# PythonOptimizers/pysparse

Measured on AMD Instinct MI355X. Metric: CSR SpMV GB/s (7-pt Poisson, % of 8 TB/s HBM peak) + PCG iters/s, higher is better.
Workload: dtype f64

## Files before the change

### pysparse_amd/csrc/psp_csr_kernels.h

```cpp

constexpr int kBlock = 256;


__global__ void build_chunk_table(int nrows, const int *__restrict__ ind, int target, int nchunks,
                                  int2 *__restrict__ tab) {
  int c = blockIdx.x * blockDim.x + threadIdx.x;
  if (c > nchunks) return;
  int r;
  if (c == nchunks) {
    r = nrows;
  } else {
    long want = (long)c * target;
    int lo = 0, hi = nrows;
    while (lo < hi) {
      int mid = lo + ((hi - lo) >> 1);
      if ((long)ind[mid] >= want)
        hi = mid;
      else
        lo = mid + 1;
    }
    r = lo;
  }
  tab[c] = make_int2(r, ind[r]);
}
// ... 1040 lines not shown
      *reinterpret_cast<d2v *>(&buf[off + 2]) = p1[st];
    }
    __builtin_amdgcn_fence(__ATOMIC_SEQ_CST, "wavefront");
    __builtin_amdgcn_wave_barrier();
#pragma unroll
    for (int m = 0; m < NP; ++m) {
      const int i = 64 * m + lane;
      if (i < nr) {
        double acc = 0.0;
        for (int k = lo[m]; k < hi[m]; k += 8) {
          double t[8];
#pragma unroll
          for (int u = 0; u < 8; ++u) {
            int id = k + u;
            id = id < WT ? id : WT - 1;
            t[u] = buf[id];
          }
#pragma unroll
          for (int u = 0; u < 8; ++u) acc += (k + u < hi[m]) ? t[u] : 0.0;
        }
        if constexpr (NTS)
          __builtin_nontemporal_store(acc, &y[r0 + i]);
        else
          y[r0 + i] = acc;
        if (dotv) dsum += dotv[r0 + i] * acc;
      }
    }
  }
  if (partials) {
    dsum = wave_sum(dsum);
    __syncthreads();
    if (lane == 0) red[wid] = dsum;
    __syncthreads();
    if (threadIdx.x == 0) {
      double t = 0.0;
#pragma unroll
      for (int i = 0; i < WPB; ++i) t += red[i];
      partials[blockIdx.x] = t;
    }
  }
}

typedef double d2u __attribute__((ext_vector_type(2), aligned(8)));

constexpr int kDiaRows = 128;
constexpr int kDiaMaxOffs = 64;
constexpr int kDiaTable = 128;
constexpr int kDiaEmpty = -0x7fffffff - 1;

struct DiaOffs {
  int o[kDiaMaxOffs];
};

__global__ void dia_offsets_kernel(int nrows, const int *__restrict__ ind, const int *__restrict__ col,
                                   int *table, int *overflow) {
  for (int r = blockIdx.x * blockDim.x + threadIdx.x; r < nrows; r += gridDim.x * blockDim.x) {
    if (*(volatile int *)overflow) return;
    int prev = -1;
    for (int k = ind[r]; k < ind[r + 1]; ++k) {
      const int c = col[k];
      if (c <= prev) {
        *overflow = 1;
        return;
      }
      prev = c;
      const int o = c - r;
      unsigned h = ((unsigned)o * 2654435761u) >> 25;
      int probes = 0;
      for (; probes < kDiaTable; ++probes, h = (h + 1) & (kDiaTable - 1)) {
        int v = *(volatile int *)(table + h);
        if (v == o) break;
        if (v == kDiaEmpty) {
          v = atomicCAS(table + h, kDiaEmpty, o);
          if (v == kDiaEmpty || v == o) break;
        }
      }
      if (probes == kDiaTable) {
        *overflow = 1;
        return;
      }
    }
  }
}

template <typename MaskT>
__global__ void dia_build_kernel(int nrows, int no, DiaOffs offs, const int *__restrict__ ind,
                                 const int *__restrict__ col, const double *__restrict__ val,
                                 double *__restrict__ valT, MaskT *__restrict__ mask) {
  for (long r = (long)blockIdx.x * blockDim.x + threadIdx.x; r < nrows; r += (long)gridDim.x * blockDim.x) {
    const long blk = r / kDiaRows;
    const int i = (int)(r % kDiaRows);
    unsigned long long m = 0;
    for (int k = ind[r]; k < ind[r + 1]; ++k) {
      const int o = col[k] - (int)r;
      int b = 0;
      while (b < no - 1 && offs.o[b] != o) ++b;
      m |= 1ull << b;
      valT[((size_t)blk * no + b) * kDiaRows + i] = val[k];
    }
    mask[r] = (MaskT)m;
  }
}

__global__ void poisson_w4_kernel(int nx, int ny, int nz, long row_lo, long nloc, int no,
                                  double *__restrict__ valT, unsigned short *__restrict__ mask) {
  const long nxy = (long)nx * ny;
// ... 480 lines not shown
      for (int u = 0; u < G; ++u) {
        const int gu = g + u < no ? g + u : no - 1;
        og[u] = offs[gu];
        v[u] = ldg<true>(reinterpret_cast<const d2v *>(vp + (size_t)gu * kDiaRows));
        const long c = r + og[u];
        const long cc = c < 0 ? 0 : (c > cmax ? cmax : c);
        const d2u t = *reinterpret_cast<const d2u *>(x + cc);
        xv[u].x = t.x;
        xv[u].y = t.y;
        edge |= cc != c;
      }
      if (edge) {
#pragma unroll
        for (int u = 0; u < G; ++u) {
          const long c = r + og[u];
          if (c < 0 || c > cmax) {
            xv[u].x = (c >= 0 && c < ncols) ? x[c] : 0.0;
            xv[u].y = (c + 1 >= 0 && c + 1 < ncols) ? x[c + 1] : 0.0;
          }
        }
      }
#pragma unroll
      for (int u = 0; u < G; ++u) {
        const double t0 = a0 + v[u].x * xv[u].x;
        const double t1 = a1 + v[u].y * xv[u].y;
        const bool live = g + u < no;
        a0 = (live && ((m0 >> (g + u)) & 1ull)) ? t0 : a0;
        a1 = (live && ((m1 >> (g + u)) & 1ull)) ? t1 : a1;
      }
    }
    if (r + 1 < nrows) {
      d2u outu;
      outu.x = a0;
      outu.y = a1;
      __builtin_nontemporal_store(outu, reinterpret_cast<d2u *>(y + r));
      if (dotv) {
        const d2u u = *reinterpret_cast<const d2u *>(dotv + r);
        dsum += u.x * a0;
        dsum += u.y * a1;
      }
    } else {
      y[r] = a0;
      if (dotv) dsum += dotv[r] * a0;
    }
  }
  if (partials) {
    dsum = wave_sum(dsum);
    if (lane == 0) red[wid] = dsum;
    __syncthreads();
    if (threadIdx.x == 0) partials[blockIdx.x] = red[0] + red[1] + red[2] + red[3];
  }
}

template <int NO, int PRE, bool XU = false>
__global__ __launch_bounds__(256) void csr_spmv_w4_pf(
    int nrows, int stripe, DiaOffs offs, const double *__restrict__ valT,
    const unsigned short *__restrict__ mask, const double *__restrict__ r, const double *__restrict__ dinv,
    double dc, const double *__restrict__ p_old, double *__restrict__ p_new, double *__restrict__ q,
    double beta, int first, double *__restrict__ partials, const psp::PcgDev *__restrict__ dstate,
    double *__restrict__ x = nullptr, double *__restrict__ scan_partials = nullptr) {
  double alpha_x = 0.0;
  bool xp = false;
  if (dstate) {
    if (dstate->status) return;
    beta = dstate->beta;
    first = dstate->it == 1;
    if constexpr (XU) {
      alpha_x = dstate->alpha_x;
      xp = dstate->xpend != 0;
    }
  }
  __shared__ double red[4];
  __shared__ double red2[4];
  double dmax = 0.0;
  const int lane = threadIdx.x & 63;
  const int wid = __builtin_amdgcn_readfirstlane(threadIdx.x >> 6);
  int vb = (int)blockIdx.x;
  if (stripe > 0) {
    const int k = vb >> 3;
    vb = ((k / stripe) * 8 + (vb & 7)) * stripe + k % stripe;
  }
  const int blk = vb * 4 + wid;
  const long row = (long)blk * kDiaRows + 2 * lane;
  double dsum = 0.0;
  if (row < nrows) {
    const unsigned mm = *reinterpret_cast<const unsigned *>(mask + row);
    const unsigned m0 = mm & 0xffffu, m1 = mm >> 16;
    const double *vp = valT + (size_t)blk * NO * kDiaRows + 2 * lane;
    d2v v[NO];
#pragma unroll
    for (int o = 0; o < NO; ++o) v[o] = ldg<true>(reinterpret_cast<const d2v *>(vp + o * kDiaRows));
    const long cmax = (long)nrows - 2;
    const long rc = row > cmax ? cmax : row;
    d2u rr[NO + 1], pp[NO + 1], dd[NO + 1];
    bool edge = rc != row;
#pragma unroll
    for (int o = 0; o <= NO; ++o) {
      const long c = o < NO ? row + offs.o[o] : row;
      const long cc = c < 0 ? 0 : (c > cmax ? cmax : c);
      rr[o] = *reinterpret_cast<const d2u *>(r + cc);
      if (!first) pp[o] = *reinterpret_cast<const d2u *>(p_old + cc);
      if constexpr (PRE == 1) dd[o] = *reinterpret_cast<const d2u *>(dinv + cc);
      edge |= cc != c;
    }
    if (edge) {
#pragma unroll
      for (int o = 0; o <= NO; ++o) {
        const long c = o < NO ? row + offs.o[o] : row;
        if (c < 0 || c > cmax) {
          const bool i0 = c >= 0 && c < nrows, i1 = c + 1 >= 0 && c + 1 < nrows;
          rr[o].x = i0 ? r[c] : 0.0;
          rr[o].y = i1 ? r[c + 1] : 0.0;
          if (!first) {
            pp[o].x = i0 ? p_old[c] : 0.0;
            pp[o].y = i1 ? p_old[c + 1] : 0.0;
          }
          if constexpr (PRE == 1) {
            dd[o].x = i0 ? dinv[c] : 0.0;
            dd[o].y = i1 ? dinv[c + 1] : 0.0;
          }
        }
      }
    }
    d2v pn[NO + 1];
#pragma unroll
    for (int o = 0; o <= NO; ++o) {
      double z0 = rr[o].x, z1 = rr[o].y;
      if constexpr (PRE == 1) {
        z0 = z0 * dd[o].x;
        z1 = z1 * dd[o].y;
      }
      if constexpr (PRE == 2) {
        z0 = z0 * dc;
        z1 = z1 * dc;
      }
      if (!first) {
        z0 = z0 + beta * pp[o].x;
        z1 = z1 + beta * pp[o].y;
      }
      pn[o].x = z0;
      pn[o].y = z1;
    }
    double a0 = 0.0, a1 = 0.0;
#pragma unroll
// ... 237 lines not shown
```

### pysparse_amd/csrc/psp_csr_select.h

```cpp
namespace psp {

static int colmask() {
#ifdef PSP_TUNING
  static const int m = [] {
    const char *e = psp::tuning_env("PSP_SPMV_COLMASK");
    return e ? atoi(e) : -1;
  }();
  return m;
#else
  return -1;
#endif
}

static int spmv_stripe() {
  static const int m = [] {
    const char *e = psp::tuning_env("PSP_SPMV_STRIPE");
    return e ? atoi(e) : -1;
  }();
  return m;
}

static int w4_auto_stripe(const psp_csr *A) {
  if (A->sym_owner) return 32;
  int plane_wgs = 0;
// ... 188 lines not shown
  if (!on || !v.w4 || A->nparts || A->nrows != A->ncols || A->nrows < 2) return PSP_OK;
  const int stripe = w4_stripe(A, v);
  const int nblk = (A->nrows + kDiaRows - 1) / kDiaRows;
  const int grid = w4_grid(nblk, stripe);
  psp::CsrExtra *ex;
  {
    std::lock_guard<std::mutex> lk(g_extra_mu);
    ex = &g_extra[A];
  }
  bool sss = false;
  if (A->sym_owner) {
    psp_sss *S = const_cast<psp_sss *>(A->sym_owner);
    PSP_TRY(ensure_sss_w4(S));
    sss = S->w4_state == 1;
  }
  if (!sss) {
    PSP_TRY(ensure_w4(A, &ex));
    if (ex->dia_state != 1 || ex->dia_no > 16) return PSP_OK;
  }
  double *pbuf = partials;
  if (partials && grid > kMaxParts) {
    PSP_TRY(ensure_big_partials(ex, grid));
    pbuf = ex->big_partials;
  }
  if (sss)
    PSP_TRY(launch_sss_w4(A->sym_owner, stripe, x, y, x, pbuf, skip, grid, 1, xdiv, xdiv_dev));
  else
    PSP_TRY(launch_w4(A, ex, stripe, 0, nblk, x, y, x, pbuf, skip, grid, 1, xdiv, xdiv_dev));
  int np = grid;
  if (pbuf != partials) {
    np = kFold;
    hipLaunchKernelGGL(fold_partials_kernel, dim3(np / 16), dim3(256), 0, stream(), pbuf, grid, partials, np);
    PSP_LAUNCH_CHECK();
  }
  if (nparts) *nparts = np;
  *available = 1;
  return PSP_OK;
}

__global__ __launch_bounds__(256) void grid_wrap_check_kernel(int n, int nx, int ny, const unsigned short *__restrict__ mask,
                                                              int *__restrict__ bad) {
  int found = 0;
  for (long r = (long)blockIdx.x * blockDim.x + threadIdx.x; r < n; r += (long)gridDim.x * blockDim.x) {
    const unsigned m = mask[r];
    const int i = (int)(r % nx), j = (int)((r / nx) % ny);
    if (((m >> 2) & 1u) && i == 0) found = 1;
    if (((m >> 4) & 1u) && i == nx - 1) found = 1;
    if (((m >> 1) & 1u) && j == 0) found = 1;
    if (((m >> 5) & 1u) && j == ny - 1) found = 1;
  }
  if (found) atomicAdd(bad, 1);
}

__global__ __launch_bounds__(256) void w4_value_range_kernel(int n, int no, const double *__restrict__ valT,
                                                             const unsigned short *__restrict__ mask, double *__restrict__ out) {
  __shared__ double smin[4][16], smax[4][16];
  double lo[16], hi[16];
  for (int o = 0; o < 16; ++o) {
    lo[o] = INFINITY;
    hi[o] = -INFINITY;
  }
  for (long r = (long)blockIdx.x * blockDim.x + threadIdx.x; r < n; r += (long)gridDim.x * blockDim.x) {
    const unsigned m = mask[r];
    const double *vp = valT + (size_t)(r / kDiaRows) * no * kDiaRows + (size_t)(r % kDiaRows);
    for (int o = 0; o < no; ++o)
      if ((m >> o) & 1u) {
        const double v = vp[(size_t)o * kDiaRows];
        lo[o] = v < lo[o] ? v : lo[o];
        hi[o] = v > hi[o] ? v : hi[o];
        if (!(v == v)) hi[o] = INFINITY, lo[o] = -INFINITY;
      }
  }
  const int lane = threadIdx.x & 63, wid = threadIdx.x >> 6;
  for (int o = 0; o < no; ++o) {
    double a = lo[o], b = hi[o];
    for (int off = 32; off > 0; off >>= 1) {
      const double a2 = __shfl_down(a, off, 64), b2 = __shfl_down(b, off, 64);
      a = a2 < a ? a2 : a;
      b = b2 > b ? b2 : b;
    }
    if (lane == 0) {
      smin[wid][o] = a;
      smax[wid][o] = b;
    }
  }
  __syncthreads();
  if ((int)threadIdx.x < no) {
    const int o = threadIdx.x;
    double a = smin[0][o], b = smax[0][o];
    for (int w = 1; w < 4; ++w) {
      a = smin[w][o] < a ? smin[w][o] : a;
      b = smax[w][o] > b ? smax[w][o] : b;
    }
    out[((size_t)blockIdx.x * no + o) * 2] = a;
    out[((size_t)blockIdx.x * no + o) * 2 + 1] = b;
  }
}

int csr_w4_view(const psp_csr *A, W4View *out, int *available) {
  *available = 0;
  Variant v = decode_variant(A->variant);
  if (A->w4_only) v.w4 = true;
  if (!v.w4 || A->nparts || A->multi || A->host || A->nrows != A->ncols || A->nrows < 2) return PSP_OK;
  psp::CsrExtra *ex;
  PSP_TRY(ensure_w4(A, &ex));
  if (ex->dia_state != 1 || ex->dia_no > 9 || !ex->dia_mask) return PSP_OK;
  out->no = ex->dia_no;
  for (int i = 0; i < 12; ++i) out->offs[i] = i < ex->dia_no ? ex->dia_offs.o[i] : 0;
  out->valT = ex->dia_val;
  out->mask = ex->dia_mask;
  out->stripe = w4_stripe(A, v);
  out->grid = w4_grid((A->nrows + kDiaRows - 1) / kDiaRows, out->stripe);
  out->grid3[0] = out->grid3[1] = out->grid3[2] = 0;
  if (ex->dia_no == 7) {
    const int *o = out->offs;
    const int s1 = o[5], s2 = o[6];
    if (ex->grid_state < 0) {
      ex->grid_state = 0;
      if (o[3] == 0 && o[4] == 1 && o[2] == -1 && o[1] == -s1 && o[0] == -s2 && s1 >= 2 && s2 % s1 == 0 && s2 / s1 >= 2 &&
          A->nrows % s2 == 0 && A->nrows / s2 >= 2) {
        int *bad = nullptr;
        PSP_HIP(hipMalloc((void **)&bad, sizeof(int)));
        PSP_HIP(hipMemsetAsync(bad, 0, sizeof(int), stream()));
        hipLaunchKernelGGL(grid_wrap_check_kernel, dim3(std::min((A->nrows + 255) / 256, 4096)), dim3(256), 0, stream(),
                           A->nrows, s1, s2 / s1, ex->dia_mask, bad);
        int hbad = 1;
        const hipError_t e1 = hipMemcpyAsync(&hbad, bad, sizeof(int), hipMemcpyDeviceToHost, stream());
        const hipError_t e2 = hipStreamSynchronize(stream());
        (void)hipFree(bad);
        if (e1 != hipSuccess || e2 != hipSuccess) return fail(PSP_ENODEV, "csr_w4_view: grid check failed");
        if (hbad == 0) {
          ex->grid_state = 1;
          ex->grid_nx = s1;
          ex->grid_ny = s2 / s1;
        }
      }
    }
    if (ex->grid_state == 1) {
      out->grid3[0] = ex->grid_nx;
      out->grid3[1] = ex->grid_ny;
      out->grid3[2] = A->nrows / (ex->grid_nx * ex->grid_ny);
    }
  }
  out->constv = 0;
  if (ex->dia_no <= 12) {
    if (ex->constv_state < 0) {
      ex->constv_state = 0;
      const int no = ex->dia_no, blocks = std::min((A->nrows + 255) / 256, 512);
      double *d = nullptr;
      PSP_HIP(hipMalloc((void **)&d, sizeof(double) * 2 * no * blocks));
      hipLaunchKernelGGL(w4_value_range_kernel, dim3(blocks), dim3(256), 0, stream(), A->nrows, no, ex->dia_val, ex->dia_mask, d);
      std::vector<double> h((size_t)2 * no * blocks);
      const hipError_t e1 = hipMemcpyAsync(h.data(), d, sizeof(double) * h.size(), hipMemcpyDeviceToHost, stream());
      const hipError_t e2 = hipStreamSynchronize(stream());
      (void)hipFree(d);
      if (e1 != hipSuccess || e2 != hipSuccess) return fail(PSP_ENODEV, "csr_w4_view: value range pass failed");
      bool all = true;
      for (int o = 0; o < no && all; ++o) {
        double lo = INFINITY, hi = -INFINITY;
        for (int b = 0; b < blocks; ++b) {
          lo = std::min(lo, h[((size_t)b * no + o) * 2]);
          hi = std::max(hi, h[((size_t)b * no + o) * 2 + 1]);
        }
        if (!(lo == hi) || std::signbit(lo) != std::signbit(hi)) all = false;
        ex->constv[o] = lo;
      }
      if (all) ex->constv_state = 1;
    }
    if (ex->constv_state == 1) {
      out->constv = 1;
      for (int o = 0; o < 12; ++o) out->cval[o] = o < ex->dia_no ? ex->constv[o] : 0.0;
    }
  }
  *available = 1;
  return PSP_OK;
}

int csr_spmv_pfx_launch(const psp_csr *A, const double *r, const double *dinv, const double *p_old, double *p_new,
                        double *q, double *x, double *partials, int *nparts, const PcgDev *dstate, int *available) {
  *available = 0;
  Variant v = decode_variant(A->variant);
  if (!v.w4 || A->nparts || A->sym_owner || A->nrows != A->ncols || A->nrows < 2 || !dstate || !partials) return PSP_OK;
  psp::CsrExtra *ex;
  PSP_TRY(ensure_w4(A, &ex));
  if (ex->dia_state != 1 || ex->dia_no > 8) return PSP_OK;
  const int stripe = w4_stripe(A, v);
  const int nblk = (A->nrows + kDiaRows - 1) / kDiaRows;
  const int grid = w4_grid(nblk, stripe);
  if (grid > kMaxParts) return PSP_OK;
  double dc = 0.0;
  const int pre = !dinv ? 0 : (dinv_constant(dinv, A->nrows, &dc) ? 2 : 1);
  double *scan = partials + 2 * (size_t)kMaxParts;
#define PSP_PFX(NO, PRE)                                                                                    \
  hipLaunchKernelGGL((csr_spmv_w4_pf<NO, PRE, true>), dim3(grid), dim3(256), 0, stream(), A->nrows, stripe, \
                     ex->dia_offs, ex->dia_val, ex->dia_mask, r, dinv, dc, p_old, p_new, q, 0.0, 0, partials, dstate, x, scan)
#define PSP_PFX_NO(NO)                \
  case NO:                            \
    if (pre == 0) PSP_PFX(NO, 0);     \
    else if (pre == 1) PSP_PFX(NO, 1); \
    else PSP_PFX(NO, 2);              \
    break
  switch (ex->dia_no) {
    PSP_PFX_NO(1); PSP_PFX_NO(2); PSP_PFX_NO(3); PSP_PFX_NO(4); PSP_PFX_NO(5); PSP_PFX_NO(6); PSP_PFX_NO(7); PSP_PFX_NO(8);
    default:
      return PSP_OK;
  }
#undef PSP_PFX_NO
#undef PSP_PFX
  PSP_LAUNCH_CHECK();
  *nparts = grid;
  *available = 1;
  return PSP_OK;
}

bool csr_spmv_has_skip(const psp_csr *A) {
  if (A->nparts) {
    for (int p = 0; p < A->nparts; ++p)
      if (A->parts[p]->nrows && !csr_spmv_has_skip(A->parts[p])) return false;
    return true;
  }
  Variant v = decode_variant(A->variant);
  if (A->w4_only) v.w4 = true;
  if (v.w4 && A->sym_owner) {
    psp_sss *S = const_cast<psp_sss *>(A->sym_owner);
    if (ensure_sss_w4(S) != PSP_OK) return false;
    if (S->w4_state == 1) return true;
  }
  if (v.w4) {
    psp::CsrExtra *ex;
    if (ensure_w4(A, &ex) != PSP_OK) return false;
    if (ex->dia_state == 1) return true;
  }
  if (!v.w2 || A->max_row_nnz > v.tile / 2) return false;
  ChunkTable *t;
  if (get_chunk_table(const_cast<psp_csr *>(A), v.tile, &t) != PSP_OK) return false;
  if (ensure_rowoff(A, t) != PSP_OK) return false;
  return t->np != 0;
}

int csr_reordered_view(const psp_csr *A, psp_csr **R, const int **perm, const int **inv) {
  *R = nullptr;
  psp::setup_mark(nullptr);
  Variant v = decode_variant(A->variant);
  if (A->nparts || A->w4_only || A->no_reorder || !(v.w1 && v.w2 && v.w3) || A->nrows != A->ncols ||
      A->max_row_nnz > v.tile / 2 || v.tile != 1024)
    return PSP_OK;
  if (v.w4) {
    if (A->sym_owner) {
      psp_sss *S = const_cast<psp_sss *>(A->sym_owner);
      PSP_TRY(ensure_sss_w4(S));
      if (S->w4_state == 1) return PSP_OK;
    }
    psp::CsrExtra *ex;
    PSP_TRY(ensure_w4(A, &ex));
    if (ex->dia_state == 1) return PSP_OK;
  }
  psp::setup_mark("first use: index-free (w4) layouts tried");
  ChunkTable *t;
  PSP_TRY(get_chunk_table(const_cast<psp_csr *>(A), v.tile, &t));
  PSP_TRY(ensure_rowoff(A, t));
// ... 663 lines not shown
```

### pysparse_amd/csrc/psp_internal.h

```cpp
#pragma once
#include <hip/hip_runtime.h>

#include <algorithm>
#include <atomic>
#include <cstdarg>
#include <cstdint>
#include <cstdio>
#include <cstdlib>
#include <initializer_list>
#include <mutex>
#include <string>
#include <vector>

#include "pysparse_hip.h"
#include "psp_recur.h"

namespace psp {

int fail(int code, const char *fmt, ...) __attribute__((format(printf, 2, 3)));
const char *tuning_env(const char *name);
void note_solve(const char *loop, int launches_per_iter, int vec_bytes_per_row, int dinv_streamed);
void note_fallback();
bool single_kernel_loops_enabled();
void setup_mark(const char *label);
// ... 371 lines not shown
namespace psp {
struct PcgDev : PcgCol {
  int status;
  int xpend;
  int stag0;
  int head_rho0;
  int head_beta0;
  int pend_maxit;
  double alpha_x;
};
struct MinresDev : MinresRot {
  double norm_r0, errtol, relres;
  int status;
  int stop;
  int skip;
  int info, iter, it_max;
};
struct KryArg {
  const KryDev *S = nullptr;
  int i0 = 0, i1 = 0, i2 = 0;
};
int op_apply(const psp_op *op, const double *x_dev, double *y_dev);
int op_apply_block(const psp_op *op, int k, const double *X, long ldx, double *Y, long ldy, const int *frozen = nullptr);
int block_args(const char *what, int nrows, int ncols, int k, const double *X, long ldx, const double *Y, long ldy);
int csr_spmm_check(const char *what, const psp_csr *A);
int csr_spmm_launch(const psp_csr *A, int k, const double *X, long ldx, double *Y, long ldy, const int *skip,
                    double *partials, long pstride, int *nparts);
int jacobi_block_dev(const psp_jacobi *K, int k, const double *X, long ldx, double *Y, long ldy);
int robust_norm2(int n, const double *v, double sq, double *out);
int csr_spmv_launch_stored(const psp_csr *A, const double *x, double *y, const double *dotv, double *partials, int *nparts,
                           const int *skip = nullptr);
void batch_trim();
int correq_apply(const psp_op *op, const double *x_dev, double *y_dev);
int bv_tdot(long n, int m, const double *V, long ld, const double *x, double *h_dev);
int bv_gemv(long n, int m, const double *V, long ld, const double *h_dev, double alpha, double beta, double *y);
int bv_rotate(long n, int j, double *V, long ld, const double *U_host, int ldu, int u0, int jn, int dst0);
int bv_rotate_again(long n, int j, double *V, long ld, int jn, int dst0);
int bv_gram(long n, int ma, const double *A, long lda, int mb, const double *B, long ldb, double *G_dev, long ldg);
int bv_resid(long n, int k, const double *AX, long ldax, const double *MX, long ldmx, const double *theta_dev,
             const int *slot_host, double *R, long ldr, double *nrm2_dev);
void bv_trim();
void sym_jacobi_eig(int j, const double *Mu, int ldm, double *s, double *U, int ldu);
int random_fill_dev(long count, unsigned long long first, double *out);
int krylov_dev(int which, const psp_op *A, const psp_op *K, int n, double *x_dev, const double *b_dev, double tol, int maxit,
               int *info, int *iter, double *relres);
inline psp_csr *op_native_csr(const psp_op *op) {
  if (!op) return nullptr;
  if (op->kind == PSP_OP_CSR) return op->csr;
  if (op->kind == PSP_OP_SSS) return op->sss->full;
  return nullptr;
}
int csr_spmv_launch(const psp_csr *A, const double *x, double *y, const double *dotv,
                    double *partials, int *nparts, const int *skip = nullptr);
int csr_spmv_pfx_launch(const psp_csr *A, const double *r, const double *dinv, const double *p_old, double *p_new,
                        double *q, double *x, double *partials, int *nparts, const PcgDev *dstate, int *available);
int csr_spmv_scaled_launch(const psp_csr *A, const double *x, double xdiv, double *y, double *partials,
                           int *nparts, int *available, const int *skip = nullptr,
                           const double *xdiv_dev = nullptr);
int csr_reordered_view(const psp_csr *A, psp_csr **R, const int **perm, const int **inv);
int reorder_gather(int n, const int *perm_dev, const double *x, double *xp, const int *skip);
bool csr_spmv_has_skip(const psp_csr *A);
int csr_spmv_overlap(const psp_csr *A, const double *x, double *y, const double *dotv,
                     double *partials, int *nparts, int row_a, int row_b, int (*wait)(void *),
                     void *ctx, const int *skip = nullptr);
int dinv_register(const double *v, long n);
void dinv_unregister(const double *v);
bool dinv_constant(const double *v, long n, double *c);
int jacobi_apply_dev(psp_jacobi *K, const double *x, double *y);
struct W4View {
  int no;
  int offs[12];
  int grid3[3];
  int constv;
  double cval[12];
  const double *valT;
  const unsigned short *mask;
  int stripe, grid;
};
int csr_w4_view(const psp_csr *A, W4View *out, int *available);
constexpr int kCoopFallback = 1;
using PcgSkFn = int(const psp_csr *A, const double *dinv, int n, double *x, double *r, double *p, double *q, double n2b,
                     double tolb, double normr0, double rho0, int maxit, int *info, int *iter, double *relres, double *hist);
using MinresSkFn = int(const psp_csr *A, const double *dinv, int n, double *x, double *v_hat, double *y, double *w, double *v,
                        double *av, double norm_r0, double beta0, double errtol, int it_max, int *info, int *iter,
                        double *relres, double *hist);
bool mid_applicable(const psp_csr *A, int n);
bool mid_minres_applicable(const psp_csr *A, int n);
bool brick_applicable(const psp_csr *A, int n);
bool brick_minres_applicable(const psp_csr *A, int n);
bool coop_applicable(const psp_csr *A, int n);
PcgSkFn pcg_mid_loop, pcg_brick_loop, pcg_coop_loop;
MinresSkFn minres_mid_loop, minres_brick_loop, minres_coop_loop;
PcgSkFn *pcg_sk_choice(const psp_csr *A, int n, bool rho_nonzero);
int sk_capacity(const void *kernel, int block, size_t lds);

template <class Ctl>
struct SkLaunch {
  const void *kernel;
  int nwg, block;
  size_t lds;
  void **args;
  Ctl **ctl;
  double **part, **hist_dev;
  std::atomic<long long> *solves = nullptr, *fallbacks = nullptr;
};
struct SkVectors {
  int n;
  double *x, *stage;
// ... 117 lines not shown
```

### pysparse_amd/csrc/psp_solvers.hip

```cpp
#include <algorithm>
#include <array>
#include <cmath>
#include <cstdlib>
#include <cstring>
#include <initializer_list>
#include <type_traits>
#include <mutex>
#include <utility>
#include <vector>

#include "psp_internal.h"

using namespace psp;

namespace psp {
int k_dot(long n, const double *x, const double *y, double *partials, int *nparts);
int k_residual(long n, const double *b, double *r, const double *dinv, double *partials, int *nparts);
int k_pupdate(long n, const double *r, const double *dinv, double beta, bool first, double *p,
              const PcgDev *st = nullptr);
int k_px_update(long n, const double *r, const double *dinv, double *p, double *x, double *partials,
                int *nparts, const PcgDev *dstate, double beta = 0.0, double alpha = 0.0, bool first = false,
                bool xpend = false);
int k_x_update(long n, double alpha, const double *p, double *x, double *partials, int *nparts,
               const PcgDev *dstate);
// ... 415 lines not shown
  const double alpha = st->rho / pq;
  st->alpha = alpha;
  st->alpha_x = alpha;
  st->stag0 = alpha == 0.0 ? 1 : 0;
  st->xpend = 1;
}

__device__ __forceinline__ void pcg_lazy_scalar_r(PcgDev *st, const double *__restrict__ scal, double *__restrict__ hist) {
  if (st->status) return;
  const int it = st->it;
  const double normr = sqrt(scal[0]);
  st->normr = normr;
  if (hist) hist[it] = normr;
  if (normr <= st->tolb) {
    pcg_finish(st, 0, it);
  } else if (it == st->maxit) {
    st->pend_maxit = 1;
    st->status = 1;
  } else {
    const double rho1 = st->rho, rho = scal[1];
    st->rho1 = rho1;
    st->rho = rho;
    st->it = it + 1;
    st->head_rho0 = rho == 0.0 ? 1 : 0;
    st->head_beta0 = 0;
    if (rho != 0.0) {
      const double beta = rho / rho1;
      st->beta = beta;
      st->head_beta0 = beta == 0.0 ? 1 : 0;
    }
  }
}

struct PcgLazyXPq : StepOf<PcgDev, 1, true> {
  static __device__ void run(PcgDev *st, const double *v0, const double *v1, double *) {
    pcg_lazy_scalar_x(st, v0);
    pcg_lazy_scalar_pq(st, v1);
  }
};
struct PcgLazyR : StepOf<PcgDev> {
  static __device__ void run(PcgDev *st, const double *v, const double *, double *hist) { pcg_lazy_scalar_r(st, v, hist); }
};

static int pcg_lazy_enabled() {
  const char *e = psp::tuning_env("PSP_PCG_LAZYX");
  return e ? atoi(e) : 1;
}

static int pcg_lazypf_mode(int n) {
  const char *e = psp::tuning_env("PSP_PCG_LAZYPF");
  return e ? atoi(e) : (n >= (1 << 21) ? 1 : 0);
}

static int pcg_async_loop_lazy(psp_csr *Acsr, const double *dinv, int n, double *x, double *r, double *p, double *p2,
                               double *q, double n2b, double tolb, double normr0, double rho0, int maxit,
                               int *info, int *iter, double *relres, double *hist, bool *folded) {
  constexpr int kBatch = 16;
  double *const P[2] = {p, p2};
  int usepf = (p2 && pcg_lazypf_mode(n)) ? 1 : 0;
  *folded = false;
  Workspace *w;
  PSP_TRY(workspace(&w));
  LoopState<PcgDev> S;
  PSP_TRY(pcg_state_begin(S, n2b, tolb, normr0, rho0, maxit, hist != nullptr));
  PcgDev *st = S.dev;
  int enqueued = 0, np = 0;
  double *stag_parts = w->partials + 2 * (size_t)kMaxParts;
  do {
    const int batch = std::max(1, std::min(kBatch, maxit - enqueued));
    for (int i = 0; i < batch; ++i) {
      int np_x = 0;
      if (usepf) {
        const int e = enqueued + i + 1;
        PSP_TRY(csr_spmv_pfx_launch(Acsr, r, dinv, P[(e - 1) & 1], P[e & 1], q, x, w->partials, &np, st, &usepf));
        np_x = np;
      }
      if (!usepf) {
        PSP_TRY(k_px_update(n, r, dinv, p, x, w->partials, &np_x, st));
        PSP_TRY(csr_spmv_launch(Acsr, p, q, p, w->partials, &np, &st->status));
      }
      PSP_TRY(reduce2_then<PcgLazyXPq>(stag_parts, np_x, w->scal_dev + 8, w->partials, np, w->scal_dev, st, 2, 0));
      PSP_TRY(k_r_update(n, 0.0, q, dinv, r, w->partials, &np, st));
      PSP_TRY(reduce_then<PcgLazyR>(w->partials, np, 2, w->scal_dev + 4, st, S.hist));
    }
    enqueued += batch;
    PSP_TRY(S.fetch());
  } while (!S.host->status);
  *folded = usepf != 0;
  PcgDev *hst = S.host;
  if (usepf) p = P[hst->it & 1];
  if (hst->xpend) {
    double s[1];
    PSP_TRY(k_x_update(n, hst->alpha_x, p, x, w->partials, &np, nullptr));
    PSP_TRY(finish_partials(stag_parts, np, 1, w->scal_dev + 8));
    PSP_TRY(fetch_scalars(w->scal_dev + 8, 1, s));
    if (hst->pend_maxit) {
      const bool stag = hst->stag0 || s[0] == 0.0;
      hst->info = stag ? -5 : -1;
      hst->iter = stag ? maxit : maxit + 1;
      hst->relres = hst->normr / hst->n2b;
    }
  }
  *info = hst->info;
  *iter = hst->iter;
  *relres = hst->relres;
  if (hist) PSP_TRY(S.fetch_hist(hist, std::min(hst->iter, maxit)));
  return PSP_OK;
}

static bool norm2_unsafe(double sq) { return !(sq >= 1e-280 && sq <= 1e280); }
static int abs_max(int n, const double *v, double *out);
static int robust_nrm2(Workspace *w, int n, const double *v, double sq, double *out) {
  if (!norm2_unsafe(sq)) {
    *out = sqrt(sq);
    return PSP_OK;
  }
  double vmax = 0.0;
  PSP_TRY(abs_max(n, v, &vmax));
  if (vmax == 0.0 || vmax != vmax || std::isinf(vmax)) {
    *out = vmax == 0.0 ? 0.0 : sqrt(sq);
    return PSP_OK;
  }
  int e = 0;
  (void)frexp(vmax, &e);
  DevVecs mem;
  double *t;
  PSP_TRY(mem.alloc(n, &t));
  PSP_HIP(hipMemcpyAsync(t, v, sizeof(double) * (size_t)n, hipMemcpyDeviceToDevice, stream()));
  PSP_TRY(k_scal(n, ldexp(1.0, -e), t));
  int np;
  double s1;
  PSP_TRY(k_dot(n, t, t, w->partials, &np));
  PSP_TRY(reduce_fetch(w, np, 1, &s1));
  *out = ldexp(sqrt(s1), e);
  return PSP_OK;
}

namespace psp {
int robust_norm2(int n, const double *v, double sq, double *out) {
  Workspace *w;
  PSP_TRY(workspace(&w));
// ... 63 lines not shown
  PSP_TRY(robust_nrm2(w, n, b, s[0], &n2b));
  if (n2b == 0.0) {
    PSP_HIP(hipMemsetAsync(x, 0, sizeof(double) * (size_t)n, stream()));
    PSP_HIP(hipStreamSynchronize(stream()));
    *info = 0;
    *relres = 0.0;
    *iter = 0;
    return PSP_OK;
  }

  *info = -1;
  const double tolb = tol * n2b;

  if (Acsr_forced)
    PSP_TRY(csr_spmv_launch(Acsr, x, r, nullptr, nullptr, nullptr));
  else
    PSP_TRY(op_apply(A, x, r));
  PSP_TRY(k_residual(n, b, r, fused ? dinv : nullptr, w->partials, &np));
  PSP_TRY(reduce_fetch(w, np, 2, s));
  double normr;
  PSP_TRY(robust_nrm2(w, n, r, s[0], &normr));
  double rho_next = s[1];
  if (hist) hist[0] = normr;

  if (normr <= tolb) {
    *info = 0;
    *relres = normr / n2b;
    *iter = 0;
    return PSP_OK;
  }

  const bool sk = single_kernel_loops_enabled();
  double dcst;
  const int dstream = (dinv && !dinv_constant(dinv, n, &dcst)) ? 1 : 0;
  if (sk && fused && maxit >= 1)
    for (const PcgSkLoop &L : pcg_sk_loops()) {
      if ((L.needs_rho && rho_next == 0.0) || !L.applicable(Acsr, n)) continue;
      const int rc = L.run(Acsr, dinv, n, x, r, p, q, n2b, tolb, normr, rho_next, maxit, info, iter, relres, hist);
      if (rc != kCoopFallback) {
        note_solve(L.name, 1, 0, dstream);
        return rc;
      }
      note_fallback();
    }
  if (fused && maxit >= 1 && pcg_async_enabled() && csr_spmv_has_skip(Acsr)) {
    if (rho_next == 0.0) {
      *info = -2;
      *iter = 1;
      *relres = normr / n2b;
      return PSP_OK;
    }
    const int lazy_mode = pcg_lazy_enabled();
    const int rl = n > (1 << 21) ? 2 : 0;
    if (lazy_mode == 2 || (lazy_mode == 1 && (n < (1 << 24) || n >= 3 * (1 << 23)))) {
      bool pf = false;
      const int rc = pcg_async_loop_lazy(Acsr, dinv, n, x, r, p, p2, q, n2b, tolb, normr, rho_next, maxit, info, iter,
                                         relres, hist, &pf);
      note_solve(pf ? "pcg_lazy_pf" : "pcg_lazy", (pf ? 4 : 5) + rl, (pf ? 56 : 64) + 16 * dstream, dstream);
      return rc;
    }
    note_solve("pcg_eager", 6 + rl, 72 + 16 * dstream, dstream);
    return pcg_async_loop(Acsr, dinv, n, x, r, p, q, n2b, tolb, normr, rho_next, maxit, info, iter, relres, hist);
  }
  note_solve("pcg_host_scalars", -1, -1, dstream);

  PcgCol c = pcg_begin(n2b, tolb, normr, maxit);
  if (maxit < 1) pcg_exit(c, -1, 1);
  while (c.it <= maxit) {
    const double *zsrc = r;
    const double *zdinv = dinv;
    if (!fused) {
      zdinv = nullptr;
      if (K) {
        PSP_TRY(op_apply(K, r, z));
        zsrc = z;
      }
      PSP_TRY(k_dot(n, r, zsrc, w->partials, &np));
      PSP_TRY(reduce_fetch(w, np, 1, s));
      rho_next = s[0];
    }
    if (pcg_head(c, rho_next)) break;
    PSP_TRY(k_pupdate(n, zsrc, zdinv, c.it == 1 ? 0.0 : c.beta, c.it == 1, p));

    if (Acsr) {
      PSP_TRY(csr_spmv_launch(Acsr, p, q, p, w->partials, &np));
    } else {
      PSP_TRY(op_apply(A, p, q));
      PSP_TRY(k_dot(n, p, q, w->partials, &np));
    }
    PSP_TRY(reduce_fetch(w, np, 1, s));
    if (pcg_alpha(c, s[0])) break;

    PSP_TRY(k_xr_update(n, c.alpha, p, q, fused ? dinv : nullptr, x, r, w->partials, &np));
    PSP_TRY(reduce_fetch(w, np, 3, s));
    rho_next = s[1];
    const int it = c.it;
    const bool over = pcg_tail(c, sqrt(s[0]), s[2] == 0.0);
    if (hist) hist[it] = c.normr;
    if (over) break;
  }
  *info = c.info;
  *iter = c.iter;
  *relres = c.relres;
  PSP_HIP(hipStreamSynchronize(stream()));
  return PSP_OK;
}


struct PermutedSystem {
  psp_csr *R = nullptr;
  const int *perm = nullptr, *inv = nullptr;
// ... 1594 lines not shown
```

Before: 6113.

## Use constant stencil coefficients in fused PCG SpMV instead of streaming matrix values

```diff
diff --git a/pysparse_amd/csrc/psp_csr_kernels.h b/pysparse_amd/csrc/psp_csr_kernels.h
--- a/pysparse_amd/csrc/psp_csr_kernels.h
+++ b/pysparse_amd/csrc/psp_csr_kernels.h
@@ -1116,6 +1116,10 @@
   int o[kDiaMaxOffs];
 };
 
+struct DiaCVals {
+  double v[8];
+};
+
 __global__ void dia_offsets_kernel(int nrows, const int *__restrict__ ind, const int *__restrict__ col,
                                    int *table, int *overflow) {
   for (int r = blockIdx.x * blockDim.x + threadIdx.x; r < nrows; r += gridDim.x * blockDim.x) {
@@ -1702,9 +1706,9 @@
   }
 }
 
-template <int NO, int PRE, bool XU = false>
+template <int NO, int PRE, bool XU = false, bool CV = false>
 __global__ __launch_bounds__(256) void csr_spmv_w4_pf(
-    int nrows, int stripe, DiaOffs offs, const double *__restrict__ valT,
+    int nrows, int stripe, DiaOffs offs, DiaCVals cv, const double *__restrict__ valT,
     const unsigned short *__restrict__ mask, const double *__restrict__ r, const double *__restrict__ dinv,
     double dc, const double *__restrict__ p_old, double *__restrict__ p_new, double *__restrict__ q,
     double beta, int first, double *__restrict__ partials, const psp::PcgDev *__restrict__ dstate,
@@ -1736,10 +1740,15 @@
   if (row < nrows) {
     const unsigned mm = *reinterpret_cast<const unsigned *>(mask + row);
     const unsigned m0 = mm & 0xffffu, m1 = mm >> 16;
-    const double *vp = valT + (size_t)blk * NO * kDiaRows + 2 * lane;
     d2v v[NO];
-#pragma unroll
-    for (int o = 0; o < NO; ++o) v[o] = ldg<true>(reinterpret_cast<const d2v *>(vp + o * kDiaRows));
+    if constexpr (CV) {
+#pragma unroll
+      for (int o = 0; o < NO; ++o) v[o].x = v[o].y = cv.v[o];
+    } else {
+      const double *vp = valT + (size_t)blk * NO * kDiaRows + 2 * lane;
+#pragma unroll
+      for (int o = 0; o < NO; ++o) v[o] = ldg<true>(reinterpret_cast<const d2v *>(vp + o * kDiaRows));
+    }
     const long cmax = (long)nrows - 2;
     const long rc = row > cmax ? cmax : row;
     d2u rr[NO + 1], pp[NO + 1], dd[NO + 1];
diff --git a/pysparse_amd/csrc/psp_csr_select.h b/pysparse_amd/csrc/psp_csr_select.h
--- a/pysparse_amd/csrc/psp_csr_select.h
+++ b/pysparse_amd/csrc/psp_csr_select.h
@@ -264,6 +264,10 @@
   if (found) atomicAdd(bad, 1);
 }
 
+__host__ __device__ inline bool value_before(double a, double b) {
+  return a < b || (a == b && __builtin_signbit(a) && !__builtin_signbit(b));
+}
+
 __global__ __launch_bounds__(256) void w4_value_range_kernel(int n, int no, const double *__restrict__ valT,
                                                              const unsigned short *__restrict__ mask, double *__restrict__ out) {
   __shared__ double smin[4][16], smax[4][16];
@@ -278,8 +282,8 @@
     for (int o = 0; o < no; ++o)
       if ((m >> o) & 1u) {
         const double v = vp[(size_t)o * kDiaRows];
-        lo[o] = v < lo[o] ? v : lo[o];
-        hi[o] = v > hi[o] ? v : hi[o];
+        lo[o] = value_before(v, lo[o]) ? v : lo[o];
+        hi[o] = value_before(hi[o], v) ? v : hi[o];
         if (!(v == v)) hi[o] = INFINITY, lo[o] = -INFINITY;
       }
   }
@@ -288,8 +292,8 @@
     double a = lo[o], b = hi[o];
     for (int off = 32; off > 0; off >>= 1) {
       const double a2 = __shfl_down(a, off, 64), b2 = __shfl_down(b, off, 64);
-      a = a2 < a ? a2 : a;
-      b = b2 > b ? b2 : b;
+      a = value_before(a2, a) ? a2 : a;
+      b = value_before(b, b2) ? b2 : b;
     }
     if (lane == 0) {
       smin[wid][o] = a;
@@ -301,12 +305,43 @@
     const int o = threadIdx.x;
     double a = smin[0][o], b = smax[0][o];
     for (int w = 1; w < 4; ++w) {
-      a = smin[w][o] < a ? smin[w][o] : a;
-      b = smax[w][o] > b ? smax[w][o] : b;
+      a = value_before(smin[w][o], a) ? smin[w][o] : a;
+      b = value_before(b, smax[w][o]) ? smax[w][o] : b;
     }
     out[((size_t)blockIdx.x * no + o) * 2] = a;
     out[((size_t)blockIdx.x * no + o) * 2 + 1] = b;
   }
+}
+
+static int w4_const_values(const psp_csr *A, psp::CsrExtra *ex, bool *constv) {
+  *constv = false;
+  if (ex->dia_state != 1 || ex->dia_no > 12) return PSP_OK;
+  if (ex->constv_state < 0) {
+    ex->constv_state = 0;
+    const int no = ex->dia_no, blocks = std::min((A->nrows + 255) / 256, 512);
+    double *d = nullptr;
+    PSP_HIP(hipMalloc((void **)&d, sizeof(double) * 2 * no * blocks));
+    hipLaunchKernelGGL(w4_value_range_kernel, dim3(blocks), dim3(256), 0, stream(), A->nrows, no, ex->dia_val, ex->dia_mask, d);
+    std::vector<double> h((size_t)2 * no * blocks);
+    const hipError_t e1 = hipMemcpyAsync(h.data(), d, sizeof(double) * h.size(), hipMemcpyDeviceToHost, stream());
+    const hipError_t e2 = hipStreamSynchronize(stream());
+    (void)hipFree(d);
+    if (e1 != hipSuccess || e2 != hipSuccess) return fail(PSP_ENODEV, "w4_const_values: value range pass failed");
+    bool all = true;
+    for (int o = 0; o < no && all; ++o) {
+      double lo = INFINITY, hi = -INFINITY;
+      for (int b = 0; b < blocks; ++b) {
+        const double bl = h[((size_t)b * no + o) * 2], bh = h[((size_t)b * no + o) * 2 + 1];
+        lo = value_before(bl, lo) ? bl : lo;
+        hi = value_before(hi, bh) ? bh : hi;
+      }
+      if (!(lo == hi) || std::signbit(lo) != std::signbit(hi)) all = false;
+      ex->constv[o] = lo;
+    }
+    if (all) ex->constv_state = 1;
+  }
+  *constv = ex->constv_state == 1;
+  return PSP_OK;
 }
 
 int csr_w4_view(const psp_csr *A, W4View *out, int *available) {
@@ -354,70 +389,80 @@
       out->grid3[2] = A->nrows / (ex->grid_nx * ex->grid_ny);
     }
   }
-  out->constv = 0;
-  if (ex->dia_no <= 12) {
-    if (ex->constv_state < 0) {
-      ex->constv_state = 0;
-      const int no = ex->dia_no, blocks = std::min((A->nrows + 255) / 256, 512);
-      double *d = nullptr;
-      PSP_HIP(hipMalloc((void **)&d, sizeof(double) * 2 * no * blocks));
-      hipLaunchKernelGGL(w4_value_range_kernel, dim3(blocks), dim3(256), 0, stream(), A->nrows, no, ex->dia_val, ex->dia_mask, d);
-      std::vector<double> h((size_t)2 * no * blocks);
-      const hipError_t e1 = hipMemcpyAsync(h.data(), d, sizeof(double) * h.size(), hipMemcpyDeviceToHost, stream());
-      const hipError_t e2 = hipStreamSynchronize(stream());
-      (void)hipFree(d);
-      if (e1 != hipSuccess || e2 != hipSuccess) return fail(PSP_ENODEV, "csr_w4_view: value range pass failed");
-      bool all = true;
-      for (int o = 0; o < no && all; ++o) {
-        double lo = INFINITY, hi = -INFINITY;
-        for (int b = 0; b < blocks; ++b) {
-          lo = std::min(lo, h[((size_t)b * no + o) * 2]);
-          hi = std::max(hi, h[((size_t)b * no + o) * 2 + 1]);
-        }
-        if (!(lo == hi) || std::signbit(lo) != std::signbit(hi)) all = false;
-        ex->constv[o] = lo;
-      }
-      if (all) ex->constv_state = 1;
-    }
-    if (ex->constv_state == 1) {
-      out->constv = 1;
-      for (int o = 0; o < 12; ++o) out->cval[o] = o < ex->dia_no ? ex->constv[o] : 0.0;
-    }
-  }
+  bool cv = false;
+  PSP_TRY(w4_const_values(A, ex, &cv));
+  out->constv = cv ? 1 : 0;
+  if (cv)
+    for (int o = 0; o < 12; ++o) out->cval[o] = o < ex->dia_no ? ex->constv[o] : 0.0;
   *available = 1;
   return PSP_OK;
 }
 
+static int pfx_layout(const psp_csr *A, psp::CsrExtra **ex, int *stripe, int *grid, bool *ok) {
+  *ok = false;
+  Variant v = decode_variant(A->variant);
+  if (!v.w4 || A->nparts || A->sym_owner || A->nrows != A->ncols || A->nrows < 2) return PSP_OK;
+  PSP_TRY(ensure_w4(A, ex));
+  if ((*ex)->dia_state != 1 || (*ex)->dia_no > 8) return PSP_OK;
+  *stripe = w4_stripe(A, v);
+  *grid = w4_grid((A->nrows + kDiaRows - 1) / kDiaRows, *stripe);
+  *ok = *grid <= kMaxParts;
+  return PSP_OK;
+}
+
+int csr_spmv_pfx_constv(const psp_csr *A, int *cv) {
+  *cv = 0;
+  psp::CsrExtra *ex;
+  int stripe, grid;
+  bool ok, c = false;
+  PSP_TRY(pfx_layout(A, &ex, &stripe, &grid, &ok));
+  if (!ok || ex->dia_no != 7) return PSP_OK;
+  PSP_TRY(w4_const_values(A, ex, &c));
+  *cv = c ? 1 : 0;
+  return PSP_OK;
+}
+
 int csr_spmv_pfx_launch(const psp_csr *A, const double *r, const double *dinv, const double *p_old, double *p_new,
-                        double *q, double *x, double *partials, int *nparts, const PcgDev *dstate, int *available) {
+                        double *q, double *x, double *partials, int *nparts, const PcgDev *dstate, int cv, int *available) {
   *available = 0;
-  Variant v = decode_variant(A->variant);
-  if (!v.w4 || A->nparts || A->sym_owner || A->nrows != A->ncols || A->nrows < 2 || !dstate || !partials) return PSP_OK;
+  if (!dstate || !partials) return PSP_OK;
   psp::CsrExtra *ex;
-  PSP_TRY(ensure_w4(A, &ex));
-  if (ex->dia_state != 1 || ex->dia_no > 8) return PSP_OK;
-  const int stripe = w4_stripe(A, v);
-  const int nblk = (A->nrows + kDiaRows - 1) / kDiaRows;
-  const int grid = w4_grid(nblk, stripe);
-  if (grid > kMaxParts) return PSP_OK;
+  int stripe, grid;
+  bool ok;
+  PSP_TRY(pfx_layout(A, &ex, &stripe, &grid, &ok));
+  if (!ok) return PSP_OK;
+  if (cv && (ex->dia_no != 7 || ex->constv_state != 1))
+    return fail(PSP_EINVAL, "csr_spmv_pfx_launch: constant-coefficient form asked for an operator that has none");
   double dc = 0.0;
   const int pre = !dinv ? 0 : (dinv_constant(dinv, A->nrows, &dc) ? 2 : 1);
   double *scan = partials + 2 * (size_t)kMaxParts;
-#define PSP_PFX(NO, PRE)                                                                                    \
-  hipLaunchKernelGGL((csr_spmv_w4_pf<NO, PRE, true>), dim3(grid), dim3(256), 0, stream(), A->nrows, stripe, \
-                     ex->dia_offs, ex->dia_val, ex->dia_mask, r, dinv, dc, p_old, p_new, q, 0.0, 0, partials, dstate, x, scan)
-#define PSP_PFX_NO(NO)                \
-  case NO:                            \
-    if (pre == 0) PSP_PFX(NO, 0);     \
-    else if (pre == 1) PSP_PFX(NO, 1); \
-    else PSP_PFX(NO, 2);              \
+  DiaCVals cvals = {};
+  if (cv)
+    for (int o = 0; o < 7; ++o) cvals.v[o] = ex->constv[o];
+#define PSP_PFX(NO, PRE, CV)                                                                                    \
+  hipLaunchKernelGGL((csr_spmv_w4_pf<NO, PRE, true, CV>), dim3(grid), dim3(256), 0, stream(), A->nrows, stripe, \
+                     ex->dia_offs, cvals, ex->dia_val, ex->dia_mask, r, dinv, dc, p_old, p_new, q, 0.0, 0, partials, dstate, x, scan)
+#define PSP_PFX_PRE(NO, CV)               \
+  do {                                    \
+    if (pre == 0) PSP_PFX(NO, 0, CV);      \
+    else if (pre == 1) PSP_PFX(NO, 1, CV); \
+    else PSP_PFX(NO, 2, CV);               \
+  } while (0)
+#define PSP_PFX_NO(NO)         \
+  case NO:                     \
+    PSP_PFX_PRE(NO, false);    \
     break
   switch (ex->dia_no) {
-    PSP_PFX_NO(1); PSP_PFX_NO(2); PSP_PFX_NO(3); PSP_PFX_NO(4); PSP_PFX_NO(5); PSP_PFX_NO(6); PSP_PFX_NO(7); PSP_PFX_NO(8);
+    PSP_PFX_NO(1); PSP_PFX_NO(2); PSP_PFX_NO(3); PSP_PFX_NO(4); PSP_PFX_NO(5); PSP_PFX_NO(6); PSP_PFX_NO(8);
+    case 7:
+      if (cv) PSP_PFX_PRE(7, true);
+      else PSP_PFX_PRE(7, false);
+      break;
     default:
       return PSP_OK;
   }
 #undef PSP_PFX_NO
+#undef PSP_PFX_PRE
 #undef PSP_PFX
   PSP_LAUNCH_CHECK();
   *nparts = grid;
diff --git a/pysparse_amd/csrc/psp_internal.h b/pysparse_amd/csrc/psp_internal.h
--- a/pysparse_amd/csrc/psp_internal.h
+++ b/pysparse_amd/csrc/psp_internal.h
@@ -447,8 +447,9 @@
 }
 int csr_spmv_launch(const psp_csr *A, const double *x, double *y, const double *dotv,
                     double *partials, int *nparts, const int *skip = nullptr);
+int csr_spmv_pfx_constv(const psp_csr *A, int *cv);
 int csr_spmv_pfx_launch(const psp_csr *A, const double *r, const double *dinv, const double *p_old, double *p_new,
-                        double *q, double *x, double *partials, int *nparts, const PcgDev *dstate, int *available);
+                        double *q, double *x, double *partials, int *nparts, const PcgDev *dstate, int cv, int *available);
 int csr_spmv_scaled_launch(const psp_csr *A, const double *x, double xdiv, double *y, double *partials,
                            int *nparts, int *available, const int *skip = nullptr,
                            const double *xdiv_dev = nullptr);
diff --git a/pysparse_amd/csrc/psp_solvers.hip b/pysparse_amd/csrc/psp_solvers.hip
--- a/pysparse_amd/csrc/psp_solvers.hip
+++ b/pysparse_amd/csrc/psp_solvers.hip
@@ -491,13 +491,20 @@
   return e ? atoi(e) : (n >= (1 << 21) ? 1 : 0);
 }
 
+static int pcg_lazypf_cv_enabled() {
+  const char *e = psp::tuning_env("PSP_PCG_LAZYPF_CV");
+  return e ? atoi(e) : 1;
+}
+
 static int pcg_async_loop_lazy(psp_csr *Acsr, const double *dinv, int n, double *x, double *r, double *p, double *p2,
                                double *q, double n2b, double tolb, double normr0, double rho0, int maxit,
-                               int *info, int *iter, double *relres, double *hist, bool *folded) {
+                               int *info, int *iter, double *relres, double *hist, int *form) {
   constexpr int kBatch = 16;
   double *const P[2] = {p, p2};
   int usepf = (p2 && pcg_lazypf_mode(n)) ? 1 : 0;
-  *folded = false;
+  int usecv = 0;
+  if (usepf && pcg_lazypf_cv_enabled()) PSP_TRY(csr_spmv_pfx_constv(Acsr, &usecv));
+  *form = 0;
   Workspace *w;
   PSP_TRY(workspace(&w));
   LoopState<PcgDev> S;
@@ -511,7 +518,7 @@
       int np_x = 0;
       if (usepf) {
         const int e = enqueued + i + 1;
-        PSP_TRY(csr_spmv_pfx_launch(Acsr, r, dinv, P[(e - 1) & 1], P[e & 1], q, x, w->partials, &np, st, &usepf));
+        PSP_TRY(csr_spmv_pfx_launch(Acsr, r, dinv, P[(e - 1) & 1], P[e & 1], q, x, w->partials, &np, st, usecv, &usepf));
         np_x = np;
       }
       if (!usepf) {
@@ -525,7 +532,7 @@
     enqueued += batch;
     PSP_TRY(S.fetch());
   } while (!S.host->status);
-  *folded = usepf != 0;
+  *form = usepf ? (usecv ? 2 : 1) : 0;
   PcgDev *hst = S.host;
   if (usepf) p = P[hst->it & 1];
   if (hst->xpend) {
@@ -695,11 +702,17 @@
     }
     const int lazy_mode = pcg_lazy_enabled();
     const int rl = n > (1 << 21) ? 2 : 0;
-    if (lazy_mode == 2 || (lazy_mode == 1 && (n < (1 << 24) || n >= 3 * (1 << 23)))) {
-      bool pf = false;
+    const bool band = n >= (1 << 24) && n < 3 * (1 << 23);
+    int cv_band = 0;
+    if (lazy_mode == 1 && band && p2 && pcg_lazypf_mode(n) && pcg_lazypf_cv_enabled())
+      PSP_TRY(csr_spmv_pfx_constv(Acsr, &cv_band));
+    if (lazy_mode == 2 || (lazy_mode == 1 && (!band || cv_band))) {
+      int form = 0;
       const int rc = pcg_async_loop_lazy(Acsr, dinv, n, x, r, p, p2, q, n2b, tolb, normr, rho_next, maxit, info, iter,
-                                         relres, hist, &pf);
-      note_solve(pf ? "pcg_lazy_pf" : "pcg_lazy", (pf ? 4 : 5) + rl, (pf ? 56 : 64) + 16 * dstream, dstream);
+                                         relres, hist, &form);
+      static const char *const names[3] = {"pcg_lazy", "pcg_lazy_pf", "pcg_lazy_pf_cv"};
+      static const int beyond[3] = {64, 56, 0};
+      note_solve(names[form], (form ? 4 : 5) + rl, beyond[form] + 16 * dstream, dstream);
       return rc;
     }
     note_solve("pcg_eager", 6 + rl, 72 + 16 * dstream, dstream);
```

New measurement: 6120, median of 2. About the same (+0.1%).
